# acids-ircam/RAVE

Hardware: AMD Instinct MI355X
Metric: audio samples/sec/GPU (RAVE v2 training step, 44.1 kHz, n_signal=65536) (higher is better)
Workload: dtype f32; 1 GPU; v2 config, batch 32 mono 44.1 kHz n_signal=65536, VAE-phase training step per GPU (--phase vae); global_batch=32, parallelism=dp1, phase=vae

## Files before the change

include/rave_hip.h:

```cpp
#ifndef RAVE_HIP_H
#define RAVE_HIP_H

#include <stddef.h>
#include <stdint.h>

#ifdef __cplusplus
extern "C" {
#endif

#define RH_VERSION 100

#define RH_OK 0
#define RH_ERR_INVALID (-1)
#define RH_ERR_UNSUPPORTED (-2)
#define RH_ERR_WORKSPACE (-3)

typedef void* rh_stream_t;

enum rh_act {
    RH_ACT_NONE = 0,
    RH_ACT_LEAKY = 1,
    RH_ACT_SNAKE = 2
};

typedef struct rh_conv1d_desc {
    int32_t batch;
    int32_t c_in;
    int32_t c_out;
    int32_t l_in;
    int32_t l_out;
    int32_t kernel;
    int32_t stride;
    int32_t dilation;
    int32_t pad_left;
    int32_t transposed;
    int32_t groups;
    int32_t inner;
    int32_t in_valid;
    int32_t act;
    float act_slope;
    int32_t out_act;
    float out_slope;
} rh_conv1d_desc;

int rh_version(void);
const char* rh_last_error(void);



int rh_weight_norm_fwd_f32(const float* v, const float* g, int64_t rows, int64_t cols, float* w,
                           float* norms, rh_stream_t stream);
int rh_weight_norm_bwd_f32(const float* dw, const float* v, const float* g, const float* norms,
                           int64_t rows, int64_t cols, float* dv, float* dg, rh_stream_t stream);
typedef struct rh_wn_bwd_item {
    const float* dw;
    const float* v;
    const float* g;
    const float* norms;
    float* dv;
    float* dg;
    int64_t rows;
    int64_t cols;
} rh_wn_bwd_item;
int rh_weight_norm_bwd_batched_f32(const rh_wn_bwd_item* items, int32_t n_items, rh_stream_t stream);
typedef struct rh_reduce_item {
    const float* part;
    float* out;
    int64_t n;
    int32_t Z;
    int32_t reserved;
} rh_reduce_item;
int rh_defer_reduce(rh_reduce_item* item);
int rh_reduce_partials_batched_f32(const rh_reduce_item* items, int32_t n_items, rh_stream_t stream);

int64_t rh_conv1d_packed_floats(const rh_conv1d_desc* d, int which);
int rh_conv1d_pack_f32(const rh_conv1d_desc* d, const float* w, float* wp_fwd, float* wp_bwd,
                       rh_stream_t stream);

int rh_conv1d_pack_wn_f32(const rh_conv1d_desc* d, const float* v, const float* g, float* norms,
                          float* scale, float* wp_fwd, float* wp_bwd, rh_stream_t stream);

int64_t rh_prep_item_bytes(void);
int64_t rh_prep_array_bytes(int32_t n);
int rh_prep_fill_item(const rh_conv1d_desc* d, const float* v, const float* g, float* norms, float* scale,
                      float* wp_fwd, float* wp_bwd, void* item_host);
int rh_prep_link(void* items_host, int32_t n, int64_t* total_rows, int64_t* total_blocks);
int rh_prep_run_f32(const void* items_dev, int32_t n, int64_t total_rows, int64_t total_blocks, rh_stream_t stream);


int rh_conv1d_fwd_f32(const rh_conv1d_desc* d, const float* x, const float* wp_fwd,
                      const float* bias, const float* snake_alpha, const float* residual,
                      float* y, void* workspace, int64_t workspace_bytes, rh_stream_t stream);
int64_t rh_conv1d_fwd_workspace_bytes(const rh_conv1d_desc* d);
int64_t rh_conv1d_bwd_data_workspace_bytes(const rh_conv1d_desc* d);
int rh_conv1d_kernel_family(const rh_conv1d_desc* d, int which, int has_bias, int has_add);
int rh_residual_unit_fused(const rh_conv1d_desc* d3, const rh_conv1d_desc* d1);
int rh_residual_unit_fwd_f32(const rh_conv1d_desc* d3, const rh_conv1d_desc* d1, const float* x, const float* wp3_fwd,
                             const float* wp1_fwd, float* h, float* y, rh_stream_t stream);

int rh_x6_uses_ranges(void);
int rh_x6_range_words(void);
int rh_x6_set_ranges(const uint32_t* in_a, const uint32_t* in_b, uint32_t* out, uint32_t* out2);
int rh_amax_f32(const float* x, int64_t n, uint32_t* slot, rh_stream_t stream);

int rh_conv1d_plan_info(const rh_conv1d_desc* d, int which, int has_bias, int has_add, int32_t* out8);
int rh_conv1d_bwd_weight_kernel_family(const rh_conv1d_desc* d);

int rh_conv1d_bwd_data_f32(const rh_conv1d_desc* d, const float* dy, const float* wp_bwd,
                           const float* x, const float* snake_alpha, const float* add, float* dx,
                           void* workspace, int64_t workspace_bytes, rh_stream_t stream);

int64_t rh_conv1d_workspace_bytes(const rh_conv1d_desc* d);
int rh_conv1d_bwd_weight_f32(const rh_conv1d_desc* d, const float* dy, const float* x,
                             const float* snake_alpha, float* dw, float* dbias, void* workspace,
                             int64_t workspace_bytes, rh_stream_t stream);
int rh_conv1d_bwd_weight_wn_f32(const rh_conv1d_desc* d, const float* dy, const float* x, const float* snake_alpha,
                                const float* v, const float* g, const float* norms, float* dw_scratch, float* dv,
                                float* dg, float* dbias, void* workspace, int64_t workspace_bytes, rh_stream_t stream);
int64_t rh_conv1d_bwd_weight_wn_fused_launches(void);


int rh_pqmf_analysis_fwd_f32(const float* x, const float* w, int32_t rows, int32_t t_len,
                             int32_t n_band, int32_t kernel, int32_t pad_left, int32_t n_frames,
                             float* y, rh_stream_t stream);
int rh_pqmf_analysis_bwd_f32(const float* dy, const float* w, int32_t rows, int32_t t_len,
                             int32_t n_band, int32_t kernel, int32_t pad_left, int32_t n_frames,
                             float* dx, rh_stream_t stream);
int rh_pqmf_synthesis_fwd_f32(const float* y, const float* w, int32_t rows, int32_t n_frames,
                              int32_t n_band, int32_t kernel, int32_t pad_left, int32_t n_out,
                              float* x, rh_stream_t stream);
int rh_pqmf_synthesis_bwd_f32(const float* dx, const float* w, int32_t rows, int32_t n_frames,
                              int32_t n_band, int32_t kernel, int32_t pad_left, int32_t n_out,
                              float* dy, rh_stream_t stream);

int rh_pqmf_fold_k1_f32(const float* in, const float* tab, int32_t rows, int32_t t_len, int32_t n_frames, int32_t o0,
                        float scale, float* out, rh_stream_t stream);
int rh_pqmf_fold_k2_f32(const float* in, const float* tab, int32_t rows, int32_t n_frames, int32_t n_out, int32_t dp,
                        float scale, float* out, rh_stream_t stream);


int rh_amp_tanh_fwd_f32(const float* x, int32_t batch, int32_t c, int32_t l, float* y,
                        rh_stream_t stream);
int rh_amp_tanh_bwd_f32(const float* dy, const float* x, int32_t batch, int32_t c, int32_t l,
                        float* dx, rh_stream_t stream);
int rh_act_fwd_f32(const float* x, const float* snake_alpha, int32_t act, float slope,
                   int32_t batch, int32_t c, int32_t l, float* y, rh_stream_t stream);
int64_t rh_snake_bwd_workspace_bytes(int32_t batch, int32_t c);
int rh_snake_bwd_f32(const float* dy, const float* x, const float* alpha, int32_t batch, int32_t c,
                     int32_t l, float* dx, float* dalpha, void* workspace, int64_t workspace_bytes,
                     rh_stream_t stream);
int rh_act_bwd_f32(const float* dy, const float* y, int32_t act, float slope, int64_t n, float* g, rh_stream_t stream);
int64_t rh_act_bwd_bias_workspace_bytes(int32_t M);
int rh_act_bwd_bias_f32(const float* dy, const float* y, int32_t act, float slope, int32_t B, int32_t M, int64_t plane, float* g,
                        float* dbias, void* workspace, int64_t workspace_bytes, rh_stream_t stream);
int rh_adain_stats_update_f32(const float* x, int64_t rows, int32_t l, const float* num_updates, float* mean_buf,
                              float* std_buf, rh_stream_t stream);
int rh_adain_transfer_f32(const float* x, int64_t rows, int32_t l, const float* mean_x, const float* std_x,
                          const float* mean_y, const float* std_y, float* y, rh_stream_t stream);
int rh_avgpool2_fwd_f32(const float* x, int64_t rows, int32_t l_in, float* y, rh_stream_t stream);
int rh_avgpool2_bwd_f32(const float* dy, int64_t rows, int32_t l_in, float* dx, rh_stream_t stream);


typedef struct rh_conv2d_desc {
    int32_t batch;
    int32_t c_in;
    int32_t c_out;
    int32_t h_in, w_in;
    int32_t h_out, w_out;
    int32_t kh, kw;
    int32_t sh, sw;
    int32_t dh, dw;
    int32_t ph, pw;
    int32_t act;
    float act_slope;
} rh_conv2d_desc;

int64_t rh_conv2d_packed_floats(const rh_conv2d_desc* d, int which);
int rh_conv2d_pack_f32(const rh_conv2d_desc* d, const float* w, float* wp_fwd, float* wp_bwd, rh_stream_t stream);
int rh_conv2d_fwd_f32(const rh_conv2d_desc* d, const float* x, const float* wp_fwd, const float* bias ,
                      float* y, rh_stream_t stream);
int rh_conv2d_bwd_data_f32(const rh_conv2d_desc* d, const float* dy, const float* y, const float* wp_bwd, float* dx,
                           rh_stream_t stream);
int rh_conv2d_plan_info(const rh_conv2d_desc* d, int32_t which, int64_t* out);
int rh_conv2d_bwd_weight_kernel_family(const rh_conv2d_desc* d);
int64_t rh_conv2d_workspace_bytes(const rh_conv2d_desc* d);
int rh_conv2d_bwd_weight_f32(const rh_conv2d_desc* d, const float* dy, const float* y, const float* x, float* dw,
                             float* dbias, void* workspace, int64_t workspace_bytes, rh_stream_t stream);


// ... 94 lines not shown
```

rave_amd/_lib.py:

```python
from __future__ import annotations

import ctypes as C
import os

import torch

_HERE = os.path.dirname(os.path.abspath(__file__))
LIB_PATH = os.environ.get("RAVE_HIP_LIB") or os.path.join(_HERE, "librave_hip.so")

ACT_NONE, ACT_LEAKY, ACT_SNAKE = 0, 1, 2


class ConvDesc(C.Structure):
    _fields_ = [
        ("batch", C.c_int32), ("c_in", C.c_int32), ("c_out", C.c_int32),
        ("l_in", C.c_int32), ("l_out", C.c_int32), ("kernel", C.c_int32),
        ("stride", C.c_int32), ("dilation", C.c_int32), ("pad_left", C.c_int32),
        ("transposed", C.c_int32), ("groups", C.c_int32), ("inner", C.c_int32),
        ("in_valid", C.c_int32), ("act", C.c_int32), ("act_slope", C.c_float),
        ("out_act", C.c_int32), ("out_slope", C.c_float),
    ]


class AdamItem(C.Structure):
    _fields_ = [("p", C.c_void_p), ("g", C.c_void_p), ("m", C.c_void_p), ("v", C.c_void_p), ("n", C.c_int64), ("step", C.c_void_p)]


class WnBwdItem(C.Structure):
    _fields_ = [("dw", C.c_void_p), ("v", C.c_void_p), ("g", C.c_void_p), ("norms", C.c_void_p), ("dv", C.c_void_p),
                ("dg", C.c_void_p), ("rows", C.c_int64), ("cols", C.c_int64)]


class ReduceItem(C.Structure):
    _fields_ = [("part", C.c_void_p), ("out", C.c_void_p), ("n", C.c_int64), ("Z", C.c_int32), ("reserved", C.c_int32)]


class LossItem(C.Structure):
    _fields_ = [("value", C.c_void_p), ("w1_dev", C.c_void_p), ("w1", C.c_float), ("w2", C.c_float)]


class FmItem(C.Structure):
    _fields_ = [("f", C.c_void_p), ("df", C.c_void_p), ("half", C.c_int64), ("w", C.c_float)]


class Conv2dDesc(C.Structure):
    _fields_ = [(n, C.c_int32) for n in (
        "batch", "c_in", "c_out", "h_in", "w_in", "h_out", "w_out", "kh", "kw", "sh", "sw", "dh", "dw", "ph", "pw",
        "act")] + [("act_slope", C.c_float)]


def _load() -> C.CDLL:
    if not os.path.exists(LIB_PATH):
        raise RuntimeError(
            f"rave_amd: {LIB_PATH} not found. Build it with `python -m rave_amd.build` "
            "(or __graft_entry__.build()). There is no CPU / PyTorch fallback for the HIP hot path.")
    lib = C.CDLL(LIB_PATH)
    P, I32, I64, F = C.c_void_p, C.c_int32, C.c_int64, C.c_float
    D = C.POINTER(ConvDesc)
    D2 = C.POINTER(Conv2dDesc)
    sig = {
        "rh_version": ([], C.c_int),
        "rh_last_error": ([], C.c_char_p),
        "rh_weight_norm_fwd_f32": ([P, P, I64, I64, P, P, P], C.c_int),
        "rh_weight_norm_bwd_f32": ([P, P, P, P, I64, I64, P, P, P], C.c_int),
        "rh_weight_norm_bwd_batched_f32": ([C.POINTER(WnBwdItem), I32, P], C.c_int),
        "rh_defer_reduce": ([C.POINTER(ReduceItem)], C.c_int),
        "rh_reduce_partials_batched_f32": ([C.POINTER(ReduceItem), I32, P], C.c_int),
        "rh_conv1d_packed_floats": ([D, C.c_int], I64),
        "rh_conv1d_pack_f32": ([D, P, P, P, P], C.c_int),
        "rh_conv1d_pack_wn_f32": ([D, P, P, P, P, P, P, P], C.c_int),
        "rh_prep_item_bytes": ([], I64),
        "rh_prep_array_bytes": ([I32], I64),
        "rh_prep_fill_item": ([D, P, P, P, P, P, P, P], C.c_int),
        "rh_prep_link": ([P, I32, C.POINTER(I64), C.POINTER(I64)], C.c_int),
        "rh_prep_run_f32": ([P, I32, I64, I64, P], C.c_int),
        "rh_conv1d_fwd_f32": ([D, P, P, P, P, P, P, P, I64, P], C.c_int),
        "rh_conv1d_bwd_data_f32": ([D, P, P, P, P, P, P, P, I64, P], C.c_int),
        "rh_conv1d_kernel_family": ([D, C.c_int, C.c_int, C.c_int], C.c_int),
        "rh_conv1d_bwd_weight_kernel_family": ([D], C.c_int),
        "rh_residual_unit_fused": ([D, D], C.c_int),
        "rh_residual_unit_fwd_f32": ([D, D, P, P, P, P, P, P], C.c_int),
        "rh_conv1d_plan_info": ([D, C.c_int, C.c_int, C.c_int, C.POINTER(C.c_int32)], C.c_int),
        "rh_conv1d_fwd_workspace_bytes": ([D], I64),
        "rh_conv1d_bwd_data_workspace_bytes": ([D], I64),
        "rh_conv1d_workspace_bytes": ([D], I64),
        "rh_conv1d_bwd_weight_f32": ([D, P, P, P, P, P, P, I64, P], C.c_int),
        "rh_conv1d_bwd_weight_wn_f32": ([D, P, P, P, P, P, P, P, P, P, P, P, I64, P], C.c_int),
        "rh_conv1d_bwd_weight_wn_fused_launches": ([], I64),
        "rh_conv2d_packed_floats": ([D2, C.c_int], I64),
        "rh_conv2d_pack_f32": ([D2, P, P, P, P], C.c_int),
        "rh_conv2d_fwd_f32": ([D2, P, P, P, P, P], C.c_int),
        "rh_conv2d_bwd_data_f32": ([D2, P, P, P, P, P], C.c_int),
        "rh_conv2d_workspace_bytes": ([D2], I64),
        "rh_conv2d_plan_info": ([D2, I32, C.POINTER(I64)], C.c_int),
        "rh_conv2d_bwd_weight_kernel_family": ([D2], C.c_int),
        "rh_conv2d_bwd_weight_f32": ([D2, P, P, P, P, P, P, I64, P], C.c_int),
        "rh_feed_batch_i16_f32": ([P, P, P, P, I32, I32, I32, P, P], C.c_int),
        "rh_vq_loss_partials": ([I64], I64),
        "rh_vq_assign_f32": ([P, P, I64, I32, I32, P, P, P, P, P], C.c_int),
        "rh_vq_assign_workspace_bytes": ([I64, I32, I32], I64),
        "rh_vq_assign_ws_f32": ([P, P, I64, I32, I32, P, P, P, P, P, I64, P], C.c_int),
        "rh_vq_ema_update_f32": ([P, P, I64, I32, I32, F, F, P, P, P, P], C.c_int),
        "rh_pqmf_analysis_fwd_f32": ([P, P, I32, I32, I32, I32, I32, I32, P, P], C.c_int),
        "rh_pqmf_analysis_bwd_f32": ([P, P, I32, I32, I32, I32, I32, I32, P, P], C.c_int),
        "rh_pqmf_synthesis_fwd_f32": ([P, P, I32, I32, I32, I32, I32, I32, P, P], C.c_int),
        "rh_pqmf_synthesis_bwd_f32": ([P, P, I32, I32, I32, I32, I32, I32, P, P], C.c_int),
        "rh_pqmf_fold_k1_f32": ([P, P, I32, I32, I32, I32, F, P, P], C.c_int),
        "rh_pqmf_fold_k2_f32": ([P, P, I32, I32, I32, I32, F, P, P], C.c_int),
        "rh_amp_tanh_fwd_f32": ([P, I32, I32, I32, P, P], C.c_int),
        "rh_amp_tanh_bwd_f32": ([P, P, I32, I32, I32, P, P], C.c_int),
        "rh_act_fwd_f32": ([P, P, I32, F, I32, I32, I32, P, P], C.c_int),
        "rh_act_bwd_f32": ([P, P, I32, F, I64, P, P], C.c_int),
        "rh_act_bwd_bias_workspace_bytes": ([I32], I64),
        "rh_act_bwd_bias_f32": ([P, P, I32, F, I32, I32, I64, P, P, P, I64, P], C.c_int),
        "rh_snake_bwd_workspace_bytes": ([I32, I32], I64),
        "rh_snake_bwd_f32": ([P, P, P, I32, I32, I32, P, P, P, I64, P], C.c_int),
        "rh_stft_frame_fwd_f32": ([P, P, I64, I32, I32, I32, I32, P, P], C.c_int),
        "rh_stft_frame_bwd_f32": ([P, P, I64, I32, I32, I32, I32, P, P], C.c_int),
        "rh_stft_frame_bwd_acc_f32": ([P, P, I64, I32, I32, I32, I32, P, I32, P], C.c_int),
        "rh_spectral_total_f32": ([P, P, I32, P, P], C.c_int),
        "rh_feature_matching_workspace_bytes": ([C.POINTER(FmItem), I32], I64),
        "rh_feature_matching_fwd_f32": ([C.POINTER(FmItem), I32, I32, P, I64, P, P, P], C.c_int),
        "rh_feature_matching_bwd_f32": ([C.POINTER(FmItem), I32, I32, P, P, P], C.c_int),
        "rh_reparam_workspace_bytes": ([], I64),
        "rh_reparam_fwd_f32": ([P, P, I32, I32, I32, P, P, P, I64, P], C.c_int),
        "rh_reparam_bwd_f32": ([P, P, P, P, I32, I32, I32, P, P], C.c_int),
        "rh_loss_combine_fwd_f32": ([C.POINTER(LossItem), I32, P, P, P], C.c_int),
        "rh_loss_combine_bwd_f32": ([C.POINTER(LossItem), I32, P, P, P], C.c_int),
        "rh_adam_step_f32": ([C.POINTER(AdamItem), I32, P, F, F, F, P, P], C.c_int),
        "rh_x6_uses_ranges": ([], C.c_int),
        "rh_x6_range_words": ([], C.c_int),
        "rh_x6_set_ranges": ([P, P, P, P], C.c_int),
        "rh_amax_f32": ([P, I64, P, P], C.c_int),
        "rh_set_kernel_events": ([P, P], C.c_int),
        "rh_kernel_events_used": ([], C.c_int),
        "rh_event_create": ([C.POINTER(C.c_void_p)], C.c_int),
        "rh_event_destroy": ([P], C.c_int),
        "rh_event_elapsed_ms": ([P, P, C.POINTER(C.c_float)], C.c_int),
        "rh_stft_loss_supported": ([I32, I32, I32, I64], C.c_int),
        "rh_stft_loss_plan_info": ([I32, I32, I64, C.POINTER(I64)], C.c_int),
        "rh_stft_loss_workspace_bytes": ([I32, I32, I64], I64),
        "rh_stft_loss_fwd_f32": ([P, P, P, P, I64, I32, I32, F, P, P, I64, P], C.c_int),
        "rh_stft_loss_finalize_all_f32": ([C.POINTER(C.c_void_p), C.POINTER(I64), I32, P, P, P, P], C.c_int),
        "rh_stft_loss_bwd_f32": ([P, P, P, P, I64, I32, I32, F, P, P, P, P, I32, P], C.c_int),
        "rh_spectral_distance_workspace_bytes": ([], I64),
        "rh_spectral_distance_fwd_f32": ([P, P, I64, F, P, P, I64, P], C.c_int),
        "rh_spectral_distance_bwd_f32": ([P, P, P, P, I64, F, P, P, I32, P], C.c_int),
        "rh_adain_stats_update_f32": ([P, I64, I32, P, P, P, P], C.c_int),
        "rh_adain_transfer_f32": ([P, I64, I32, P, P, P, P, P, P], C.c_int),
        "rh_avgpool2_fwd_f32": ([P, I64, I32, P, P], C.c_int),
        "rh_avgpool2_bwd_f32": ([P, I64, I32, P, P], C.c_int),
    }
    for name, (args, res) in sig.items():
        fn = getattr(lib, name)
        fn.argtypes = args
        fn.restype = res
    return lib


lib = _load()


# ... 13 lines not shown
```

rave_amd/csrc/conv_wgrad.hip:

```cpp
#include <atomic>
#include <cstdlib>
#include <mutex>
#include "conv_params.hpp"

namespace {

template <int TM, int TN, int WM, int WN>
__global__ __launch_bounds__(WM* WN * 64) void wgrad_kernel(const WgradP p) {
    constexpr int BM = TM * WM * 32, BN = TN * WN * 32;
    constexpr int NW = WM * WN;
    extern __shared__ __attribute__((aligned(16))) float smem[];
    float* r_lds = smem;
    float* s_lds = smem + BM * p.pr;

    const int tid = threadIdx.x, lane = tid & 63, wave = tid >> 6;
    const int j = lane & 31, kh = lane >> 5;
    const int wm = wave / WN, wn = wave - wm * WN;
    const int m0 = blockIdx.y * BM, col0 = blockIdx.x * BN, z = blockIdx.z;
    const int ncols = p.C * p.T;
    const int inner = p.inner, is = p.is;
    const int c_lo = col0 / p.T;

    int sb[TN], ar[TM];
#pragma unroll
// ... 584 lines not shown
        const unsigned long long rb = 4ull * p.B * p.M * (unsigned long long)p.r_row;
        const unsigned long long sbytes = 4ull * p.B * p.C * (unsigned long long)p.s_row;
        const bool ok = p.r_act != RH_ACT_SNAKE && p.s_act != RH_ACT_SNAKE && rb < 0x7fffffffull &&
                        sbytes < 0x7fffffffull && w.rk * p.inner <= 64 && w.total_chunks < 32768;
        if (ok) {
            p.nc_max = (BN - 1) / p.T + 2;
            if (p.nc_max > p.C) p.nc_max = p.C;
            const int s_width = ((w.rk - 1) * p.is + (p.maxoff - p.minoff) + 1) * p.inner;
            static const int novec = [] { const char* e = getenv("RH_WGRAD_NOVEC"); return e ? atoi(e) : 0; }();
            p.vec = !novec && p.inner == 1 && (w.rk % 4) == 0 && (p.r_row % 4) == 0 && (p.s_row % 4) == 0 &&
                    ((uintptr_t)p.R % 16) == 0 && ((uintptr_t)p.S % 16) == 0;
            if (p.vec) {
                p.pr = w.rk + 4;
                p.ps = ((s_width + 3) & ~3) + 4;
                if ((p.ps & 31) == 0) p.ps += 4;
                const int ni_r = rh_cdiv(BM * (p.pr >> 2), 64 * WM * WN);
                const int ni_s = rh_cdiv(p.nc_max * (p.ps >> 2), 64 * WM * WN);
                if (ni_r > 12 || ni_s > 12) p.vec = 0;
            }
            if (!p.vec) {
                p.ps = s_width | 1;
                p.pr = (w.rk * p.inner) | 1;
            }
            p.magic_pr = magic_of(p.pr);
            p.magic_lpr_r = magic_of(p.pr >> 2);
            p.magic_lpr_s = magic_of(p.ps >> 2);
            p.r_floats = (BM * p.pr + 255) & ~255;
            p.s_floats = (p.nc_max * p.ps + 255) & ~255;
            p.stage_floats = p.r_floats + p.s_floats;
            p.magic_ps = magic_of(p.ps);
            p.magic_cpb = magic_of(w.chunks_per_b);
            p.r_bytes = (unsigned)rb;
            p.s_bytes = (unsigned)sbytes;
            const size_t lds = sizeof(float) * 2 * (size_t)p.stage_floats;
            if (lds <= 160 * 1024 && (unsigned)p.s_floats < (1u << 15)) {
                dim3 grid(w.ct, w.mt, w.Z);
                auto go = [&](auto kern) {
                    static std::once_flag once;
                    std::call_once(once, [&] { (void)hipFuncSetAttribute(reinterpret_cast<const void*>(kern), hipFuncAttributeMaxDynamicSharedMemorySize, 160 * 1024); });
                    rh_launch_main(kern, grid, dim3(WM * WN * 64), lds, stream, p);
                };
                if (p.r_act == RH_ACT_LEAKY) go(wgrad_dma_kernel<TM, TN, WM, WN, true, false>);
                else if (p.s_act == RH_ACT_LEAKY) go(wgrad_dma_kernel<TM, TN, WM, WN, false, true>);
                else go(wgrad_dma_kernel<TM, TN, WM, WN, false, false>);
                return rh_check_launch("conv1d_bwd_weight(dma)");
            }
        }
    }
    p.pr = (w.rk * p.inner) | 1;
    p.ps = (((w.rk - 1) * p.is + (p.maxoff - p.minoff) + 1) * p.inner) | 1;
    p.nc_max = (BN - 1) / p.T + 2;
    if (p.nc_max > p.C) p.nc_max = p.C;
    const size_t lds = sizeof(float) * ((size_t)BM * p.pr + (size_t)p.nc_max * p.ps);
    RH_REQUIRE(lds <= 160 * 1024, RH_ERR_UNSUPPORTED, "conv1d_bwd_weight: tile needs %zu B of LDS", lds);
    auto kern = wgrad_kernel<TM, TN, WM, WN>;
    static std::once_flag once;
    std::call_once(once, [&] {
        (void)hipFuncSetAttribute(reinterpret_cast<const void*>(kern),
                                  hipFuncAttributeMaxDynamicSharedMemorySize, 160 * 1024);
    });
    dim3 grid(w.ct, w.mt, w.Z);
    rh_launch_main(kern, grid, dim3(WM * WN * 64), lds, stream, p);
    return rh_check_launch("conv1d_bwd_weight");
}

}

int64_t rh_wgrad_x6_workspace(const WgradP& w);
int rh_wgrad_x6_launch(const WgradP& w, float* dw, float* rsum_out, void* ws, hipStream_t stream, bool* used, int* left_z,
                       const unsigned* r_range, const unsigned* s_range);
int rh_reduce_wn_bwd_launch(const float* part, int Z, long M, long N, const float* v, const float* g, const float* norms,
                            float* dv, float* dg, hipStream_t stream, bool* used);

extern "C" int rh_conv1d_bwd_weight_kernel_family(const rh_conv1d_desc* d) {
    if (!d || d->batch <= 0) return 0;
    WgradP p{};
    fill(d, &p);
    if (rh_smallc_wgrad_eligible(d)) return 2;
    alignas(16) static const float dummy[4] = {0.f, 0.f, 0.f, 0.f};
    p.R = dummy; p.S = dummy;
    return d->act != RH_ACT_SNAKE && rh_wgrad_x6_workspace(p) >= 0 ? 1 : 0;
}

int64_t rh_wgrad_workspace(const rh_conv1d_desc* d) {
    WgradP p{};
    fill(d, &p);
    const int64_t bias = rh_bias_grad_workspace(d->c_out);
    if (rh_smallc_wgrad_eligible(d)) return bias + rh_smallc_wgrad_workspace(d);
    int64_t x6 = -1;
    if (d->act != RH_ACT_SNAKE) {
        x6 = rh_wgrad_x6_workspace(p);
        if (x6 >= 0 && !RH_X6_F16) return bias + x6;
    }
    const WPlan w = plan(p);
    const int64_t f32 = w.Z <= 1 ? 0 : (int64_t)w.Z * p.M * p.C * p.T * (int64_t)sizeof(float);
    return bias + (x6 > f32 ? x6 : f32);
}

extern "C" int rh_weight_norm_bwd_f32(const float* dw, const float* v, const float* g, const float* norms, int64_t rows,
                                      int64_t cols, float* dv, float* dg, rh_stream_t stream);

thread_local rh_reduce_item* g_defer_item = nullptr;
extern "C" int rh_defer_reduce(rh_reduce_item* item) {
    g_defer_item = item;
    if (item) *item = rh_reduce_item{};
    return RH_OK;
}

extern "C" int rh_reduce_partials_batched_f32(const rh_reduce_item* items, int32_t n_items, rh_stream_t stream) {
    RH_REQUIRE(n_items >= 0 && (n_items == 0 || items), RH_ERR_INVALID, "reduce_partials_batched: bad arguments");
    for (int i0 = 0; i0 < n_items; i0 += kReduceBatch) {
        ReduceTable tb{};
        long blocks = 0;
        for (int i = i0; i < n_items && i < i0 + kReduceBatch; ++i) {
            const rh_reduce_item& q = items[i];
            if (q.Z <= 0 || q.n <= 0) continue;
            RH_REQUIRE(q.part && q.out, RH_ERR_INVALID, "reduce_partials_batched: null pointer in item %d", i);
            const int k = tb.items++;
            tb.part[k] = q.part; tb.out[k] = q.out; tb.Z[k] = q.Z;
            tb.vec4[k] = reduce_is_vec4(q.part, q.out, q.n, q.Z) ? 1 : 0;
            tb.n[k] = tb.vec4[k] ? q.n / 4 : q.n;
            tb.blk_begin[k] = blocks;
            blocks += tb.vec4[k] ? rh_cdiv64(tb.n[k], 256) : rh_cdiv64(q.n, 64);
        }
        if (tb.items == 0) continue;
        tb.blk_begin[tb.items] = blocks;
        RH_REQUIRE(blocks < 0x7fffffffl, RH_ERR_UNSUPPORTED, "reduce_partials_batched: too many workgroups");
        hipLaunchKernelGGL(reduce_partials_batched_kernel, dim3((unsigned)blocks), dim3(256), 0, (hipStream_t)stream, tb);
        if (int e = rh_check_launch("reduce_partials_batched")) return e;
    }
    return RH_OK;
}

RhWgradArmed rh_wgrad_take_armed(bool may_defer) {
    RhWgradArmed a{may_defer ? g_defer_item : nullptr, nullptr, nullptr};
    g_defer_item = nullptr;
    rh_take_ranges(&a.dy_range, &a.x_range, nullptr, nullptr);
    return a;
}

int rh_wgrad_run(const rh_conv1d_desc* d, const float* dy, const float* x, const float* alpha,
                 float* dw, float* dbias, void* ws, int64_t ws_bytes, hipStream_t stream, const RhWgradArmed& armed,
                 const RhWnTail* tail) {
    rh_reduce_item* const defer = tail ? nullptr : armed.defer;
    WgradP p{};
    fill(d, &p);
    const unsigned* const dy_range = armed.dy_range;
    const unsigned* const x_range = armed.x_range;
    const bool have_ranges = !RH_X6_F16 || (dy_range && x_range);
    auto through_dw = [&](int e) {
        if (e || !tail) return e;
        return rh_weight_norm_bwd_f32(dw, tail->v, tail->g, tail->norms, p.M, (int64_t)p.C * p.T, tail->dv, tail->dg, (rh_stream_t)stream);
    };
    if (!d->transposed) { p.R = dy; p.S = x; p.r_alpha = nullptr; p.s_alpha = alpha; }
    else                { p.R = x; p.S = dy; p.r_alpha = alpha; p.s_alpha = nullptr; }
    const long nw = (long)p.M * p.C * p.T;
    const int64_t bias_ws = rh_bias_grad_workspace(d->c_out);
    if (rh_smallc_wgrad_eligible(d)) {
        const int64_t need = rh_smallc_wgrad_workspace(d);
        RH_REQUIRE(ws && ws_bytes >= need, RH_ERR_WORKSPACE, "conv1d_bwd_weight: workspace %lld B < %lld B",
                   (long long)ws_bytes, (long long)need);
        return through_dw(rh_smallc_wgrad(d, dy, x, dw, dbias, ws, stream));
    }
    const bool x6_path = have_ranges && d->act != RH_ACT_SNAKE && p.B > 0 && p.r_row > 0 && rh_wgrad_x6_workspace(p) >= 0;
    const bool fuse_bias = x6_path && !d->transposed && dbias != nullptr;
    if (dbias && d->batch > 0 && !fuse_bias) {
// ... 115 lines not shown
```

rave_amd/csrc/conv_wgrad_x6.hip:

```cpp
#include <cstdlib>
#include <mutex>
#include "conv_params.hpp"

namespace {

typedef unsigned u32x4 __attribute__((ext_vector_type(4)));
constexpr unsigned kOOB = 0x80000000u;

struct Wx6P {
    const float* R;
    const float* S;
    float* out;
    float* rsum;
    int B, M, C, T, N;
    int r_row, s_row, s_valid, is;
    float r_slope, s_slope;
    int steps_per_b;
    int total_steps, steps_per_z;
    unsigned r_bytes, s_bytes;
    int minoff, maxoff;
    int p8, cpb, chmax;
    const unsigned* r_range;
    const unsigned* s_range;
    int off[kMaxTaps];
};

typedef u32x4 u32x4_u __attribute__((aligned(2)));

__device__ __forceinline__ void emit(const float (&v)[8], float slope, float sc, u32x4* dst, int piece_stride) {
#if RH_X6_F16
    u32x4 hi, lo;
#pragma unroll
    for (int k = 0; k < 4; ++k) {
        float a = v[2 * k] * sc, b = v[2 * k + 1] * sc;
        a = rh_max1(a, a * slope);
        b = rh_max1(b, b * slope);
        const rh_h2 h = rh_h2_split(a, b);
        hi[k] = h.hi; lo[k] = h.lo;
    }
    dst[0] = hi;
    dst[piece_stride] = lo;
#else
    unsigned h[3][8];
#pragma unroll
    for (int i = 0; i < 8; ++i) {
        const float x = rh_max1(v[i], v[i] * slope);
        rh_bf3_split(x, h[0][i], h[1][i], h[2][i]);
    }
#pragma unroll
    for (int s3 = 0; s3 < 3; ++s3) {
        u32x4 pk;
#pragma unroll
        for (int k = 0; k < 4; ++k) pk[k] = __builtin_amdgcn_perm(h[s3][2 * k + 1], h[s3][2 * k], 0x07060302u);
        dst[s3 * piece_stride] = pk;
    }
#endif
}

constexpr int kKS = 2;

template <int TM, int WM, int WN, bool AV, bool PART, bool PL>
__global__ __launch_bounds__(256, 2) void wgrad_x6_kernel(const Wx6P p) {
    static_assert(WM * WN == 4, "four waves");
    constexpr int BM = 32 * TM * WM, BN = 64 * WN;
    constexpr int A_GS = kX6P * BM + 4, B_GS = kX6P * BN + 4;
    constexpr int A_UNITS = 2 * A_GS, B_UNITS = 2 * B_GS;
    constexpr int OCT = 2 * kKS;
    constexpr int NA = (OCT * BM + 255) / 256;
    constexpr int NB = PL ? ((BN / 2 + 2) * 7 + 255) / 256 : (OCT * BN + 255) / 256;
    extern __shared__ __attribute__((aligned(16))) unsigned char smem_raw[];
    u32x4* const a_st = reinterpret_cast<u32x4*>(smem_raw);
    u32x4* const b_st = a_st + kKS * A_UNITS;

    const int tid = threadIdx.x, lane = tid & 63;
    const int wave = __builtin_amdgcn_readfirstlane(tid >> 6);
    const int j = lane & 31, g = lane >> 5;
    const int wm = wave / WN, wn = wave - wm * WN;
    const int m0 = blockIdx.y * BM, n0 = blockIdx.x * BN, z = blockIdx.z;

    const auto r_rsrc = __builtin_amdgcn_make_buffer_rsrc(const_cast<float*>(p.R), 0, p.r_bytes, 0x00020000);
    const auto s_rsrc = __builtin_amdgcn_make_buffer_rsrc(const_cast<float*>(p.S), 0, p.s_bytes, 0x00020000);
#if RH_X6_F16
    int inv_r, inv_s;
    const float rsc = __uint_as_float(rh_x6_scale_bits(rh_range_max(p.r_range), &inv_r));
    const float ssc = __uint_as_float(rh_x6_scale_bits(rh_range_max(p.s_range), &inv_s));
    const float osc = __uint_as_float(rh_x6_unscale_bits(inv_r, inv_s));
#else
    const float rsc = 1.f, ssc = 1.f, osc = 1.f;
#endif

    unsigned aoff[NA], boff[NB];
    int adst[NA], bdst[NB], apos[NA], bp0[NB];
#pragma unroll
    for (int q = 0; q < NA; ++q) {
        const int u = tid + 256 * q;
        const int o = u % OCT, m = u / OCT;
        const bool ok = m < BM && m0 + m < p.M;
        adst[q] = m < BM ? (o >> 1) * A_UNITS + (o & 1) * A_GS + m : -1;
        apos[q] = 8 * o;
        aoff[q] = ok ? (unsigned)(((m0 + m) * p.r_row + 8 * o) * 4) : kOOB;
    }
    const int c_lo = PL ? n0 / p.T : 0;
    const int n_ch = PL ? min(p.N - 1, n0 + BN - 1) / p.T - c_lo + 1 : 0;
    const unsigned b_piece = PL ? (unsigned)(p.chmax * p.cpb) : 0u;
// ... 110 lines not shown
    __syncthreads();
    const int arow = g * A_GS + wm * TM * 32 + j;
    const int bcol = g * B_GS + wn * 64 + j;
    const int live_tn = !PART ? 2 : (n0 + wn * 64 >= p.N ? 0 : (n0 + wn * 64 + 32 >= p.N ? 1 : 2));
    const bool live1 = live_tn >= 1, live2 = live_tn == 2;
    for (int s = 0; s < nst; ++s) {
        const bool more = s + 1 < nst;
        if (more) load(st0 + s + 1);
        if (live1) {
#pragma unroll
            for (int kb = 0; kb < kKS; ++kb) {
                const u32x4* al = a_st + kb * A_UNITS + arow;
                const u32x4* bl = b_st + kb * B_UNITS + bcol;
                constexpr int SA[RH_X6_NPROD] = RH_X6_SA, SB[RH_X6_NPROD] = RH_X6_SB;
                rh_x6_frag afr[TM][kX6P];
#pragma unroll
                for (int tm = 0; tm < TM; ++tm)
#pragma unroll
                    for (int s3 = 0; s3 < kX6P; ++s3) afr[tm][s3] = __builtin_bit_cast(rh_x6_frag, al[s3 * BM + tm * 32]);
                if constexpr (PL) {
                    const unsigned char* bimg = reinterpret_cast<const unsigned char*>(b_st) + (kb * 16 + g * 8) * 2;
                    rh_x6_frag bfr[2][kX6P];
#pragma unroll
                    for (int tn = 0; tn < 2; ++tn)
#pragma unroll
                        for (int s3 = 0; s3 < kX6P; ++s3)
                            bfr[tn][s3] = __builtin_bit_cast(rh_x6_frag, *reinterpret_cast<const u32x4_u*>(bimg + bcolb[tn] + (unsigned)s3 * b_piece));
#pragma unroll
                    for (int q = 0; q < RH_X6_NPROD; ++q)
#pragma unroll
                        for (int tm = 0; tm < TM; ++tm) {
                            acc[tm][0] = RH_X6_MFMA(afr[tm][SA[q]], bfr[0][SB[q]], acc[tm][0]);
                            if (live2) acc[tm][1] = RH_X6_MFMA(afr[tm][SA[q]], bfr[1][SB[q]], acc[tm][1]);
                        }
                } else {
                    rh_x6_frag bfr[2][kX6P];
#pragma unroll
                    for (int tn = 0; tn < 2; ++tn)
#pragma unroll
                        for (int s3 = 0; s3 < kX6P; ++s3) bfr[tn][s3] = __builtin_bit_cast(rh_x6_frag, bl[s3 * BN + tn * 32]);
#pragma unroll
                    for (int q = 0; q < RH_X6_NPROD; ++q)
#pragma unroll
                        for (int tm = 0; tm < TM; ++tm) {
                            acc[tm][0] = RH_X6_MFMA(afr[tm][SA[q]], bfr[0][SB[q]], acc[tm][0]);
                            if (live2) acc[tm][1] = RH_X6_MFMA(afr[tm][SA[q]], bfr[1][SB[q]], acc[tm][1]);
                        }
                }
            }
        }
        __syncthreads();
        if (more) convert();
        __syncthreads();
    }

    if (want_rsum) {
#pragma unroll
        for (int q = 0; q < NA; ++q) {
            float v = rs_acc[q];
            v += __shfl_xor(v, 1, 64);
            v += __shfl_xor(v, 2, 64);
            const int u = tid + 256 * q;
            const int m = u / OCT;
            if ((u % OCT) == 0 && m < BM && m0 + m < p.M) p.rsum[(long)z * p.M + m0 + m] = v;
        }
    }
    float* __restrict__ outz = p.out + (long)z * p.M * p.N;
#pragma unroll
    for (int tn = 0; tn < 2; ++tn) {
        const int col = n0 + wn * 64 + tn * 32 + j;
        if (col >= p.N) continue;
#pragma unroll
        for (int tm = 0; tm < TM; ++tm) {
            const int mb = m0 + (wm * TM + tm) * 32 + 4 * g;
#pragma unroll
            for (int r = 0; r < 16; ++r) {
                const int m = mb + (r & 3) + 8 * (r >> 2);
                if (m < p.M) outz[(long)m * p.N + col] = RH_X6_F16 ? acc[tm][tn][r] * osc : acc[tm][tn][r];
            }
        }
    }
}

struct Wx6Plan {
    int tm, wm, rt, ct, Z, steps_per_z;
    int planes;
    size_t lds;
};

bool plan_wx6(const WgradP& w, Wx6P* p, Wx6Plan* pl, const unsigned* r_range, const unsigned* s_range) {
    const char* e = getenv("RH_WGRAD_X6");
    if (e && atoi(e) == 0) return false;
    if (RH_X6_F16 && (!r_range || !s_range)) return false;
    if (w.inner != 1 || w.T > kMaxTaps || w.B <= 0 || w.r_row <= 0) return false;
    if ((w.r_act != RH_ACT_NONE && w.r_act != RH_ACT_LEAKY) || (w.s_act != RH_ACT_NONE && w.s_act != RH_ACT_LEAKY)) return false;
    if ((w.r_act == RH_ACT_LEAKY && !(w.r_slope >= 0.f && w.r_slope <= 1.f)) || (w.s_act == RH_ACT_LEAKY && !(w.s_slope >= 0.f && w.s_slope <= 1.f))) return false;
    if (w.M < 32 || (long)w.C * w.T < 64) return false;
    static const int force = [] { const char* e2 = getenv("RH_WGRAD_X6_ALL"); return e2 ? atoi(e2) : 0; }();
    if (!force && w.M <= 64 && w.r_row > 1024) return false;
    const unsigned long long rb = 4ull * w.B * w.M * (unsigned long long)w.r_row;
    const unsigned long long sb = 4ull * w.B * w.C * (unsigned long long)w.s_row;
    if (rb >= 0x7fffffffull || sb >= 0x7fffffffull) return false;
    *p = Wx6P{};
    p->R = w.R; p->S = w.S;
    p->B = w.B; p->M = w.M; p->C = w.C; p->T = w.T; p->N = w.C * w.T;
    p->r_row = w.r_row; p->s_row = w.s_row; p->s_valid = w.s_valid; p->is = w.is;
    p->r_slope = w.r_act == RH_ACT_LEAKY ? w.r_slope : 1.f;
    p->s_slope = w.s_act == RH_ACT_LEAKY ? w.s_slope : 1.f;
    p->steps_per_b = rh_cdiv(w.r_row, 16 * kKS);
    p->total_steps = w.B * p->steps_per_b;
    p->r_bytes = (unsigned)rb; p->s_bytes = (unsigned)sb;
    p->minoff = w.minoff; p->maxoff = w.maxoff;
    p->r_range = r_range; p->s_range = s_range;
    for (int t = 0; t < w.T; ++t) p->off[t] = w.off[t];
    const int Mp = (w.M + 31) & ~31;
    pl->tm = (Mp % 128 == 0 && Mp >= 256 && w.T > 1) ? 2 : (Mp % 96 == 0 ? 3 : (Mp % 64 == 0 ? 2 : 1));
    static const int tm_env = [] { const char* e2 = getenv("RH_WGRAD_X6_TM"); return e2 ? atoi(e2) : 0; }();
    if (tm_env >= 1 && tm_env <= 3) pl->tm = tm_env;
    pl->wm = Mp >= 64 * pl->tm ? 2 : 1;
    const int BM = 32 * pl->tm * pl->wm, BN = 64 * (4 / pl->wm);
    pl->rt = rh_cdiv(w.M, BM);
    pl->ct = rh_cdiv(p->N, BN);
    {
        const char* pe = getenv("RH_WGRAD_X6_PLANES");
        const bool on = pe ? pe[0] == '1' : Mp <= 96;
        const int reach = w.maxoff - w.minoff;
        const int p8 = (32 + reach + 7) / 8;
        pl->planes = on && pl->tm >= 2 && w.is == 1 && w.T >= 2 && reach >= 0 && p8 <= 7 && 4l * (w.s_row + 64) * w.C * w.B < 0x7fffffffl;
        p->p8 = p8;
        p->cpb = 16 * ((p8 & 1) ? p8 : p8 + 1);
        p->chmax = BN / w.T + 2;
    }
    const size_t a_bytes = (size_t)kKS * 2 * (kX6P * BM + 4) * 16;
    pl->lds = a_bytes + (pl->planes ? (size_t)kX6P * p->chmax * p->cpb + 32 : (size_t)kKS * 2 * (kX6P * BN + 4) * 16);
    const char* te = getenv("RH_WGRAD_X6_BLOCKS");
    const int target_env = te ? atoi(te) : 0;
    const int target = target_env > 0 ? target_env : (target_env < 0 ? (pl->tm == 2 ? 768 : 512) : 512);
    int Z = rh_cdiv(target, pl->rt * pl->ct);
    const int zmax = p->total_steps / 4 > 0 ? p->total_steps / 4 : 1;
    if (Z > zmax) Z = zmax;
    if (Z < 1) Z = 1;
    pl->steps_per_z = rh_cdiv(p->total_steps, Z);
    pl->Z = rh_cdiv(p->total_steps, pl->steps_per_z);
    p->steps_per_z = pl->steps_per_z;
    return true;
}

template <int TM, int WM, bool AV, bool PART, bool PL>
void go4(const Wx6P& p, const Wx6Plan& pl, hipStream_t stream) {
    auto kern = wgrad_x6_kernel<TM, WM, 4 / WM, AV, PART, PL>;
    static std::once_flag once;
    std::call_once(once, [&] {
        (void)hipFuncSetAttribute(reinterpret_cast<const void*>(kern), hipFuncAttributeMaxDynamicSharedMemorySize, 160 * 1024);
    });
    rh_launch_main(kern, dim3(pl.ct, pl.rt, pl.Z), dim3(256), pl.lds, stream, p);
}

template <int TM, int WM, bool AV, bool PART>
void go3(const Wx6P& p, const Wx6Plan& pl, hipStream_t stream) {
    if constexpr (TM >= 2) {
        if (pl.planes) return go4<TM, WM, AV, PART, true>(p, pl, stream);
    }
    go4<TM, WM, AV, PART, false>(p, pl, stream);
}

template <int TM, int WM, bool AV>
void go2(const Wx6P& p, const Wx6Plan& pl, hipStream_t stream) {
    constexpr int TPW = 2 * (4 / WM);
    if (rh_cdiv(p.N, 32) % TPW != 0) go3<TM, WM, AV, true>(p, pl, stream);
    else go3<TM, WM, AV, false>(p, pl, stream);
}

template <int TM, int WM>
void go(const Wx6P& p, const Wx6Plan& pl, hipStream_t stream) {
    if (p.r_row % 4 == 0 && ((uintptr_t)p.R & 15) == 0) go2<TM, WM, true>(p, pl, stream);
    else go2<TM, WM, false>(p, pl, stream);
}

}

int64_t rh_wgrad_x6_workspace(const WgradP& w) {
    Wx6P p;
    Wx6Plan pl{};
    static const unsigned any_range[kRangeSlotWords] = {};
    if (!plan_wx6(w, &p, &pl, any_range, any_range)) return -1;
    return (pl.Z > 1 ? (int64_t)pl.Z * w.M * w.C * w.T : 0) * (int64_t)sizeof(float) + (int64_t)pl.Z * w.M * (int64_t)sizeof(float);
}

int rh_wgrad_x6_launch(const WgradP& w, float* dw, float* rsum_out, void* ws, hipStream_t stream, bool* used, int* left_z,
                       const unsigned* r_range, const unsigned* s_range) {
    *used = false;
    if (left_z) *left_z = 0;
    Wx6P p;
    Wx6Plan pl{};
    if (!plan_wx6(w, &p, &pl, r_range, s_range)) return RH_OK;
    p.out = pl.Z > 1 ? (float*)ws : dw;
    float* const rs_part = (float*)ws + (pl.Z > 1 ? (long)pl.Z * w.M * w.C * w.T : 0);
    p.rsum = rsum_out ? (pl.Z > 1 ? rs_part : rsum_out) : nullptr;
    if (pl.wm == 1) {
        if (pl.tm == 1) go<1, 1>(p, pl, stream);
        else if (pl.tm == 2) go<2, 1>(p, pl, stream);
        else go<3, 1>(p, pl, stream);
    } else {
        if (pl.tm == 1) go<1, 2>(p, pl, stream);
        else if (pl.tm == 2) go<2, 2>(p, pl, stream);
        else go<3, 2>(p, pl, stream);
    }
    if (int e = rh_check_launch("conv1d_bwd_weight_x6")) return e;
    *used = true;
    if (pl.Z > 1) {
        if (left_z) *left_z = pl.Z;
        else if (int e = rh_reduce_partials_launch((const float*)ws, dw, (long)w.M * w.C * w.T, pl.Z, stream, "conv1d_bwd_weight_reduce")) return e;
        if (rsum_out) return rh_reduce_partials_launch(rs_part, rsum_out, w.M, pl.Z, stream, "conv1d_bwd_bias_reduce");
    }
    return RH_OK;
}
```

Before: 242.9 million samples/s.

## Add wide single-tile x6 weight-gradient kernel for 96-row, narrow-column convolutions

Adds a specialised weight-gradient kernel for convolutions with 65–96 output rows and at most 288 columns. Each block covers all rows with TM=3 and the full column extent using a variable number of waves (3/4/6/9), double-buffering LDS stages. The split across blocks then comes only from the reduction (Z) dimension. The aim is to stop reloading the A operand across several column and row tiles and to cut launch-grid fragmentation, at the cost of larger LDS use per block and possibly lower occupancy. It also adds a plan-info query entry point and environment toggles.

```diff
diff --git a/include/rave_hip.h b/include/rave_hip.h
--- a/include/rave_hip.h
+++ b/include/rave_hip.h
@@ -105,6 +105,7 @@
 
 int rh_conv1d_plan_info(const rh_conv1d_desc* d, int which, int has_bias, int has_add, int32_t* out8);
 int rh_conv1d_bwd_weight_kernel_family(const rh_conv1d_desc* d);
+int rh_conv1d_bwd_weight_plan_info(const rh_conv1d_desc* d, int32_t* out4);
 
 int rh_conv1d_bwd_data_f32(const rh_conv1d_desc* d, const float* dy, const float* wp_bwd,
                            const float* x, const float* snake_alpha, const float* add, float* dx,
diff --git a/rave_amd/_lib.py b/rave_amd/_lib.py
--- a/rave_amd/_lib.py
+++ b/rave_amd/_lib.py
@@ -78,6 +78,7 @@
         "rh_conv1d_bwd_data_f32": ([D, P, P, P, P, P, P, P, I64, P], C.c_int),
         "rh_conv1d_kernel_family": ([D, C.c_int, C.c_int, C.c_int], C.c_int),
         "rh_conv1d_bwd_weight_kernel_family": ([D], C.c_int),
+        "rh_conv1d_bwd_weight_plan_info": ([D, C.POINTER(C.c_int32)], C.c_int),
         "rh_residual_unit_fused": ([D, D], C.c_int),
         "rh_residual_unit_fwd_f32": ([D, D, P, P, P, P, P, P], C.c_int),
         "rh_conv1d_plan_info": ([D, C.c_int, C.c_int, C.c_int, C.POINTER(C.c_int32)], C.c_int),
diff --git a/rave_amd/csrc/conv_wgrad.hip b/rave_amd/csrc/conv_wgrad.hip
--- a/rave_amd/csrc/conv_wgrad.hip
+++ b/rave_amd/csrc/conv_wgrad.hip
@@ -690,6 +690,20 @@
     return d->act != RH_ACT_SNAKE && rh_wgrad_x6_workspace(p) >= 0 ? 1 : 0;
 }
 
+bool rh_wgrad_x6_plan_info(const WgradP& w, int32_t* out4);
+
+extern "C" int rh_conv1d_bwd_weight_plan_info(const rh_conv1d_desc* d, int32_t* out4) {
+    if (!d || !out4) return RH_ERR_INVALID;
+    for (int i = 0; i < 4; ++i) out4[i] = 0;
+    if (d->batch <= 0 || rh_conv1d_bwd_weight_kernel_family(d) != 1) return RH_OK;
+    WgradP p{};
+    fill(d, &p);
+    alignas(16) static const float dummy[4] = {0.f, 0.f, 0.f, 0.f};
+    p.R = dummy; p.S = dummy;
+    (void)rh_wgrad_x6_plan_info(p, out4);
+    return RH_OK;
+}
+
 int64_t rh_wgrad_workspace(const rh_conv1d_desc* d) {
     WgradP p{};
     fill(d, &p);
diff --git a/rave_amd/csrc/conv_wgrad_x6.hip b/rave_amd/csrc/conv_wgrad_x6.hip
--- a/rave_amd/csrc/conv_wgrad_x6.hip
+++ b/rave_amd/csrc/conv_wgrad_x6.hip
@@ -20,6 +20,8 @@
     unsigned r_bytes, s_bytes;
     int minoff, maxoff;
     int p8, cpb, chmax;
+    int av;
+    unsigned b_stage;
     const unsigned* r_range;
     const unsigned* s_range;
     int off[kMaxTaps];
@@ -296,9 +298,222 @@
     }
 }
 
+template <int NW, bool PL>
+__global__ __launch_bounds__(64 * NW) void wgrad_x6_wide_kernel(const Wx6P p) {
+    constexpr int TM = 3, BM = 32 * TM, BN = 32 * NW, NT = 64 * NW, ST = 2;
+    constexpr int A_GS = kX6P * BM + 4, B_GS = kX6P * BN + 4;
+    constexpr int A_UNITS = 2 * A_GS, B_UNITS = 2 * B_GS;
+    constexpr int OCT = 2 * kKS;
+    constexpr int NA = (OCT * BM + NT - 1) / NT;
+    constexpr int NB = 2;
+    extern __shared__ __attribute__((aligned(16))) unsigned char smem_raw[];
+    u32x4* const a_st = reinterpret_cast<u32x4*>(smem_raw);
+    unsigned char* const b_st = smem_raw + (size_t)ST * kKS * A_UNITS * 16;
+
+    const int tid = threadIdx.x, lane = tid & 63;
+    const int wave = __builtin_amdgcn_readfirstlane(tid >> 6);
+    const int j = lane & 31, g = lane >> 5;
+    const int z = blockIdx.x;
+
+    const auto r_rsrc = __builtin_amdgcn_make_buffer_rsrc(const_cast<float*>(p.R), 0, p.r_bytes, 0x00020000);
+    const auto s_rsrc = __builtin_amdgcn_make_buffer_rsrc(const_cast<float*>(p.S), 0, p.s_bytes, 0x00020000);
+#if RH_X6_F16
+    int inv_r, inv_s;
+    const float rsc = __uint_as_float(rh_x6_scale_bits(rh_range_max(p.r_range), &inv_r));
+    const float ssc = __uint_as_float(rh_x6_scale_bits(rh_range_max(p.s_range), &inv_s));
+    const float osc = __uint_as_float(rh_x6_unscale_bits(inv_r, inv_s));
+#else
+    const float rsc = 1.f, ssc = 1.f, osc = 1.f;
+#endif
+
+    unsigned aoff[NA], boff[NB];
+    int adst[NA], bdst[NB], apos[NA], bp0[NB];
+#pragma unroll
+    for (int q = 0; q < NA; ++q) {
+        const int u = tid + NT * q;
+        const int o = u % OCT, m = u / OCT;
+        adst[q] = m < BM ? (o >> 1) * A_UNITS + (o & 1) * A_GS + m : -1;
+        apos[q] = 8 * o;
+        aoff[q] = m < p.M ? (unsigned)((m * p.r_row + 8 * o) * 4) : kOOB;
+    }
+    const unsigned b_piece = PL ? (unsigned)(p.chmax * p.cpb) : 0u;
+    const int nb_tasks = PL ? p.C * p.p8 : OCT * BN;
+#pragma unroll
+    for (int q = 0; q < NB; ++q) {
+        const int u = (NT - 1 - tid) + NT * q;
+        if constexpr (PL) {
+            const int ch = u / p.p8, o = u - ch * p.p8;
+            const bool ok = ch < p.C;
+            bdst[q] = ok ? ch * p.cpb + o * 16 : -1;
+            bp0[q] = p.minoff + 8 * o;
+            boff[q] = ok ? (unsigned)((ch * p.s_row + bp0[q]) * 4) : kOOB;
+        } else {
+            const int o = u % OCT, col = u / OCT;
+            const int cc = col / p.T, t = col - cc * p.T;
+            const bool ok = col < p.N;
+            bdst[q] = ok ? ((o >> 1) * B_UNITS + (o & 1) * B_GS + col) * 16 : -1;
+            bp0[q] = 8 * o * p.is + (ok ? p.off[t] : 0);
+            boff[q] = ok ? (unsigned)((cc * p.s_row + bp0[q]) * 4) : kOOB;
+        }
+    }
+    const int col = 32 * wave + j;
+    const bool live = 32 * wave < p.N;
+    unsigned bcolb = 0u;
+    if constexpr (PL) {
+        if (col < p.N) {
+            const int cc = col / p.T, t = col - cc * p.T;
+            bcolb = (unsigned)(cc * p.cpb + (p.off[t] - p.minoff) * 2);
+        }
+    }
+
+    f32x16 acc[TM];
+#pragma unroll
+    for (int tm = 0; tm < TM; ++tm)
+#pragma unroll
+        for (int r = 0; r < 16; ++r) acc[tm][r] = 0.f;
+
+    constexpr int SPAN = 16 * kKS;
+    float ra[NA][8], rb[NB][8];
+    auto load = [&](int st) {
+        const int b = st / p.steps_per_b;
+        const int n = (st - b * p.steps_per_b) * SPAN;
+        const unsigned rs = (unsigned)((b * p.M * p.r_row + n) * 4);
+        const unsigned ss = (unsigned)((b * p.C * p.s_row + n * p.is) * 4);
+        const bool r_tail = n + SPAN > p.r_row;
+        const bool s_edge = PL ? (n + p.minoff < 0 || n + p.minoff + 8 * p.p8 > p.s_valid || r_tail)
+                               : (n * p.is + p.minoff < 0 || (n + SPAN - 1) * p.is + p.maxoff >= p.s_valid || r_tail);
+#pragma unroll
+        for (int q = 0; q < NA; ++q) {
+            if (NT > OCT * BM && 64 * wave >= OCT * BM) continue;
+            const unsigned base = aoff[q] == kOOB ? kOOB : aoff[q] + rs;
+            if (p.av) {
+#pragma unroll
+                for (int h = 0; h < 2; ++h) {
+                    unsigned off = base == kOOB ? kOOB : base + 16u * h;
+                    if (r_tail) off = n + apos[q] + 4 * h < p.r_row ? off : kOOB;
+                    const u32x4 v = __builtin_bit_cast(u32x4, __builtin_amdgcn_raw_buffer_load_b128(r_rsrc, off, 0, 0));
+#pragma unroll
+                    for (int i = 0; i < 4; ++i) ra[q][4 * h + i] = __uint_as_float(v[i]);
+                }
+            } else {
+#pragma unroll
+                for (int i = 0; i < 8; ++i) {
+                    unsigned off = base == kOOB ? kOOB : base + 4u * i;
+                    if (r_tail) off = n + apos[q] + i < p.r_row ? off : kOOB;
+                    ra[q][i] = __builtin_bit_cast(float, __builtin_amdgcn_raw_buffer_load_b32(r_rsrc, off, 0, 0));
+                }
+            }
+        }
+#pragma unroll
+        for (int q = 0; q < NB; ++q) {
+            if (NT * q >= nb_tasks) continue;
+            const unsigned base = boff[q] == kOOB ? kOOB : boff[q] + ss;
+#pragma unroll
+            for (int i = 0; i < 8; ++i) {
+                unsigned off = base == kOOB ? kOOB : base + 4u * (unsigned)(i * p.is);
+                if (s_edge) {
+                    const int pos = n * p.is + bp0[q] + i * p.is;
+                    off = (pos >= 0 && pos < p.s_valid) ? off : kOOB;
+                }
+                rb[q][i] = __builtin_bit_cast(float, __builtin_amdgcn_raw_buffer_load_b32(s_rsrc, off, 0, 0));
+            }
+        }
+    };
+    const bool want_rsum = p.rsum != nullptr;
+    float rs_acc[NA];
+#pragma unroll
+    for (int q = 0; q < NA; ++q) {
+        rs_acc[q] = 0.f;
+#pragma unroll
+        for (int i = 0; i < 8; ++i) ra[q][i] = 0.f;
+    }
+    auto convert = [&](int stage) {
+        if (want_rsum) {
+#pragma unroll
+            for (int q = 0; q < NA; ++q)
+                rs_acc[q] += ((ra[q][0] + ra[q][1]) + (ra[q][2] + ra[q][3])) + ((ra[q][4] + ra[q][5]) + (ra[q][6] + ra[q][7]));
+        }
+        u32x4* const as = a_st + stage * (kKS * A_UNITS);
+        unsigned char* const bs = b_st + stage * p.b_stage;
+#pragma unroll
+        for (int q = 0; q < NA; ++q)
+            if (adst[q] >= 0) emit(ra[q], p.r_slope, rsc, as + adst[q], BM);
+#pragma unroll
+        for (int q = 0; q < NB; ++q) {
+            if (NT * q >= nb_tasks || bdst[q] < 0) continue;
+            emit(rb[q], p.s_slope, ssc, reinterpret_cast<u32x4*>(bs + bdst[q]), PL ? (int)(b_piece >> 4) : BN);
+        }
+    };
+    auto multiply = [&](int stage) {
+        const u32x4* const as = a_st + stage * (kKS * A_UNITS) + g * A_GS + j;
+        const unsigned char* const bs = b_st + stage * p.b_stage;
+#pragma unroll
+        for (int kb = 0; kb < kKS; ++kb) {
+            constexpr int SA[RH_X6_NPROD] = RH_X6_SA, SB[RH_X6_NPROD] = RH_X6_SB;
+            const u32x4* al = as + kb * A_UNITS;
+            rh_x6_frag afr[TM][kX6P], bfr[kX6P];
+#pragma unroll
+            for (int tm = 0; tm < TM; ++tm)
+#pragma unroll
+                for (int s3 = 0; s3 < kX6P; ++s3) afr[tm][s3] = __builtin_bit_cast(rh_x6_frag, al[s3 * BM + tm * 32]);
+#pragma unroll
+            for (int s3 = 0; s3 < kX6P; ++s3) {
+                if constexpr (PL)
+                    bfr[s3] = __builtin_bit_cast(rh_x6_frag, *reinterpret_cast<const u32x4_u*>(bs + (kb * 16 + g * 8) * 2 + bcolb + (unsigned)s3 * b_piece));
+                else
+                    bfr[s3] = __builtin_bit_cast(rh_x6_frag, reinterpret_cast<const u32x4*>(bs)[kb * B_UNITS + g * B_GS + s3 * BN + col]);
+            }
+#pragma unroll
+            for (int q = 0; q < RH_X6_NPROD; ++q)
+#pragma unroll
+                for (int tm = 0; tm < TM; ++tm) acc[tm] = RH_X6_MFMA(afr[tm][SA[q]], bfr[SB[q]], acc[tm]);
+        }
+    };
+
+    const int st0 = z * p.steps_per_z;
+    const int nst = min(p.steps_per_z, p.total_steps - st0);
+    if (nst > 0) {
+        load(st0);
+        convert(0);
+    }
+    __syncthreads();
+    for (int s = 0; s < nst; ++s) {
+        const bool more = s + 1 < nst;
+        if (more) load(st0 + s + 1);
+        if (live) multiply(s & 1);
+        if (more) convert((s + 1) & 1);
+        __syncthreads();
+    }
+
+    if (want_rsum) {
+#pragma unroll
+        for (int q = 0; q < NA; ++q) {
+            float v = rs_acc[q];
+            v += __shfl_xor(v, 1, 64);
+            v += __shfl_xor(v, 2, 64);
+            const int u = tid + NT * q;
+            const int m = u / OCT;
+            if ((u % OCT) == 0 && m < p.M) p.rsum[(long)z * p.M + m] = v;
+        }
+    }
+    if (col < p.N) {
+        float* __restrict__ outz = p.out + (long)z * p.M * p.N;
+#pragma unroll
+        for (int tm = 0; tm < TM; ++tm) {
+#pragma unroll
+            for (int r = 0; r < 16; ++r) {
+                const int m = tm * 32 + 4 * g + (r & 3) + 8 * (r >> 2);
+                if (m < p.M) outz[(long)m * p.N + col] = RH_X6_F16 ? acc[tm][r] * osc : acc[tm][r];
+            }
+        }
+    }
+}
+
 struct Wx6Plan {
     int tm, wm, rt, ct, Z, steps_per_z;
     int planes;
+    int nw;
+    int own_z;
     size_t lds;
 };
 
@@ -347,10 +562,32 @@
     }
     const size_t a_bytes = (size_t)kKS * 2 * (kX6P * BM + 4) * 16;
     pl->lds = a_bytes + (pl->planes ? (size_t)kX6P * p->chmax * p->cpb + 32 : (size_t)kKS * 2 * (kX6P * BN + 4) * 16);
+    int z_tiles = pl->rt * pl->ct;
+    pl->nw = 0; pl->own_z = 0;
+    {
+        const char* we = getenv("RH_WGRAD_X6_WIDE");
+        const int wide = we ? atoi(we) : 1;
+        if (wide != 0 && !getenv("RH_WGRAD_X6_PLANES") && !(tm_env >= 1 && tm_env <= 3) && w.M > 64 && w.M <= 96 && p->N <= 288) {
+            const int tiles = rh_cdiv(p->N, 32);
+            pl->nw = tiles <= 3 ? 3 : (tiles <= 4 ? 4 : (tiles <= 6 ? 6 : 9));
+            const int reach = w.maxoff - w.minoff;
+            const int p8 = (32 + reach + 7) / 8;
+            pl->planes = w.is == 1 && w.T >= 2 && reach >= 0 && p8 <= 7 && 4l * (w.s_row + 64) * w.C * w.B < 0x7fffffffl;
+            p->chmax = w.C;
+            p->av = w.r_row % 4 == 0 && ((uintptr_t)w.R & 15) == 0;
+            p->b_stage = (unsigned)(pl->planes ? ((size_t)kX6P * p->chmax * p->cpb + 32 + 15) / 16 * 16
+                                               : (size_t)kKS * 2 * (kX6P * 32 * pl->nw + 4) * 16);
+            pl->lds = 2 * ((size_t)kKS * 2 * (kX6P * 96 + 4) * 16 + p->b_stage);
+            pl->own_z = wide != 2;
+            if (pl->own_z) z_tiles = 1;
+            pl->tm = 3; pl->wm = 1; pl->rt = 1; pl->ct = 1;
+        }
+    }
     const char* te = getenv("RH_WGRAD_X6_BLOCKS");
     const int target_env = te ? atoi(te) : 0;
-    const int target = target_env > 0 ? target_env : (target_env < 0 ? (pl->tm == 2 ? 768 : 512) : 512);
-    int Z = rh_cdiv(target, pl->rt * pl->ct);
+    const int wide_target = pl->nw == 9 && pl->own_z ? 256 : 512;
+    const int target = target_env > 0 ? target_env : (target_env < 0 ? (pl->tm == 2 ? 768 : 512) : wide_target);
+    int Z = rh_cdiv(target, z_tiles);
     const int zmax = p->total_steps / 4 > 0 ? p->total_steps / 4 : 1;
     if (Z > zmax) Z = zmax;
     if (Z < 1) Z = 1;
@@ -385,6 +622,22 @@
     else go3<TM, WM, AV, false>(p, pl, stream);
 }
 
+template <int NW, bool PL>
+void go_wide2(const Wx6P& p, const Wx6Plan& pl, hipStream_t stream) {
+    auto kern = wgrad_x6_wide_kernel<NW, PL>;
+    static std::once_flag once;
+    std::call_once(once, [&] {
+        (void)hipFuncSetAttribute(reinterpret_cast<const void*>(kern), hipFuncAttributeMaxDynamicSharedMemorySize, 160 * 1024);
+    });
+    rh_launch_main(kern, dim3(pl.Z), dim3(64 * NW), pl.lds, stream, p);
+}
+
+template <int NW>
+void go_wide(const Wx6P& p, const Wx6Plan& pl, hipStream_t stream) {
+    if (pl.planes) go_wide2<NW, true>(p, pl, stream);
+    else go_wide2<NW, false>(p, pl, stream);
+}
+
 template <int TM, int WM>
 void go(const Wx6P& p, const Wx6Plan& pl, hipStream_t stream) {
     if (p.r_row % 4 == 0 && ((uintptr_t)p.R & 15) == 0) go2<TM, WM, true>(p, pl, stream);
@@ -399,6 +652,18 @@
     static const unsigned any_range[kRangeSlotWords] = {};
     if (!plan_wx6(w, &p, &pl, any_range, any_range)) return -1;
     return (pl.Z > 1 ? (int64_t)pl.Z * w.M * w.C * w.T : 0) * (int64_t)sizeof(float) + (int64_t)pl.Z * w.M * (int64_t)sizeof(float);
+}
+
+bool rh_wgrad_x6_plan_info(const WgradP& w, int32_t* out4) {
+    Wx6P p;
+    Wx6Plan pl{};
+    static const unsigned any_range[kRangeSlotWords] = {};
+    if (!plan_wx6(w, &p, &pl, any_range, any_range)) return false;
+    out4[0] = pl.nw > 0 ? pl.nw : 4;
+    out4[1] = pl.rt * pl.ct * pl.Z;
+    out4[2] = pl.Z;
+    out4[3] = pl.planes;
+    return true;
 }
 
 int rh_wgrad_x6_launch(const WgradP& w, float* dw, float* rsum_out, void* ws, hipStream_t stream, bool* used, int* left_z,
@@ -411,7 +676,12 @@
     p.out = pl.Z > 1 ? (float*)ws : dw;
     float* const rs_part = (float*)ws + (pl.Z > 1 ? (long)pl.Z * w.M * w.C * w.T : 0);
     p.rsum = rsum_out ? (pl.Z > 1 ? rs_part : rsum_out) : nullptr;
-    if (pl.wm == 1) {
+    if (pl.nw > 0) {
+        if (pl.nw == 3) go_wide<3>(p, pl, stream);
+        else if (pl.nw == 4) go_wide<4>(p, pl, stream);
+        else if (pl.nw == 6) go_wide<6>(p, pl, stream);
+        else go_wide<9>(p, pl, stream);
+    } else if (pl.wm == 1) {
         if (pl.tm == 1) go<1, 1>(p, pl, stream);
         else if (pl.tm == 2) go<2, 1>(p, pl, stream);
         else go<3, 1>(p, pl, stream);
```

Result: faster. 247.1 million samples/s, median of 6 (+1.7%).
